# ocrickard/piper-swift

Measured on AMD Instinct MI355X. Metric: audio-sec/wall-sec (RTF^-1) with ms/utterance, Piper VITS en_GB-medium geometry, scale-bench factor, higher is better.
Workload: dtype f32; 1 GPU; medium factor=8: 112 ids, 336 frames, 86016 samples (3.901 s audio) per utterance, 1 utterance per step per GPU; factor=8, phoneme_count=112, frames=336, samples=86016, parallelism=utterance-replicas x1 (one-shot RCCL weight broadcast)

## Files before the change

piper-swift_amd/csrc/conv_lean.hip:

```cpp
#include "conv.h"

namespace ph {
namespace {

typedef float f32x4 __attribute__((ext_vector_type(4)));

struct LeanArgs {
  const float *x, *w, *bias, *res, *skip;
  float *y, *y2;
  const int* len_ptr;
  int len_mul, Lin, Lout, Cout, y_len, nsteps, wn_c;
  int x_row_bytes;
  int x_base_bytes;
  int q_stride;
  int kk_sign;
  int out_ch_base, out_ch_sign;
  int x_batch_bytes;
  long long x_bs, y_bs, y2_bs;
  long long bias_bs;
};

__device__ __forceinline__ float bload(__amdgpu_buffer_rsrc_t r, int voff, int soff) {
  return __builtin_bit_cast(float, __builtin_amdgcn_raw_buffer_load_b32(r, voff, soff, 0));
}

template <int NQ, int MODE>
__global__ __launch_bounds__(512) void conv_k1_kernel(const LeanArgs a, const int nch) {
  __shared__ float red_all[2 * 8 * 4 * 64];
  const int lane = threadIdx.x & 63;
  const int wave = __builtin_amdgcn_readfirstlane((int)(threadIdx.x >> 6));
  const int mt = blockIdx.x, n = blockIdx.z;
  const int lim = a.len_ptr ? min(a.len_ptr[n] * a.len_mul, a.Lout) : a.Lout;
  int ch = blockIdx.y;
// ... 575 lines not shown
    a.out_ch_base = 0; a.out_ch_sign = 1;
    a.x_batch_bytes = (int)(c.x_batch_stride * 4);
    a.x_bs = c.x_batch_stride; a.y_bs = c.y_batch_stride; a.y2_bs = 0; a.bias_bs = 0;
    LnArgs ln{c.ln_gamma, c.ln_beta, c.ln_out, c.ln_eps};
    const dim3 grid((unsigned)ceil_div(c.Cout, 16), (unsigned)ceil_div(c.Lout, 16), (unsigned)c.N);
    if (c.K == 1) hipLaunchKernelGGL((conv_k1_ln_kernel<6>), grid, dim3(512), 0, s, a, ln);
    else if (c.epilogue == EPI_RELU) hipLaunchKernelGGL((conv_k3_ln_kernel<6, EPI_RELU>), grid, dim3(512), 0, s, a, ln);
    else hipLaunchKernelGGL((conv_k3_ln_kernel<6, EPI_STORE>), grid, dim3(512), 0, s, a, ln);
    hipError_t e = hipGetLastError();
    if (e != hipSuccess) PH_FAIL(PIPER_HIP_ERR_LAUNCH, "conv_lean (LayerNorm) launch failed: %s", hipGetErrorString(e));
    return 1;
  }
  if (c.K == 3 && c.w8 && c.Cin == 768 && c.prologue == PRO_NONE && c.epilogue == EPI_STORE && !c.stats_out && !c.gate && c.dil == 1 && c.padL == 1 &&
      c.Lin == c.Lout && c.in_ch_sign == 1 && c.in_ch_base == 0 && c.out_ch_sign == 1 && c.out_ch_base == 0 && c.N <= 65535 && !c.bias_batch_stride) {
    const int mt8 = (int)ceil_div(c.Cout, 8), nch = (int)ceil_div(c.Lout, 16);
    if ((int64_t)mt8 * nch * c.N <= 2 * (int64_t)ctx->num_cus && nch <= 65535 && c.x_batch_stride * 4 < 0x7fffffffLL) {
      LeanArgs a;
      a.x = c.x; a.w = c.w8; a.bias = c.bias; a.res = c.res; a.skip = nullptr; a.y = c.y; a.y2 = nullptr;
      a.len_ptr = c.len_ptr; a.len_mul = c.len_mul;
      a.Lin = c.Lin; a.Lout = c.Lout; a.Cout = c.Cout; a.y_len = c.y_len; a.wn_c = 0; a.nsteps = (c.Cin / 4) * c.K;
      a.x_row_bytes = c.Lin * 4; a.kk_sign = 1; a.x_base_bytes = 0; a.q_stride = 16 * c.Lin; a.out_ch_base = 0; a.out_ch_sign = 1;
      a.x_batch_bytes = (int)(c.x_batch_stride * 4); a.x_bs = c.x_batch_stride; a.y_bs = c.y_batch_stride; a.y2_bs = 0; a.bias_bs = 0;
      const int w_bytes = mt8 * a.nsteps * 128;
      constexpr int NQ = 24;
      const size_t lds = (size_t)(8 * 4 * 64 + 8 * (4 * NQ) * 20) * sizeof(float);
      static bool configured[kMaxDevices] = {};
      if (lds_optin_needed(configured))
        (void)hipFuncSetAttribute((const void*)conv_k3_r8_kernel<NQ>, hipFuncAttributeMaxDynamicSharedMemorySize, 160 * 1024);
      hipLaunchKernelGGL((conv_k3_r8_kernel<NQ>), dim3((unsigned)mt8, (unsigned)nch, (unsigned)c.N), dim3(512), lds, s, a, w_bytes);
      hipError_t e = hipGetLastError();
      if (e != hipSuccess) PH_FAIL(PIPER_HIP_ERR_LAUNCH, "conv_lean (8-row tiles) launch failed: %s", hipGetErrorString(e));
      return 1;
    }
  }
  if (c.K != 1 || c.prologue != PRO_NONE || c.stats_out || !c.w16) return 0;
  if (c.epilogue != EPI_STORE && c.epilogue != EPI_RSUB && c.epilogue != EPI_WN_RES_SKIP && c.epilogue != EPI_WN_SKIP_LAST) return 0;
  if ((c.epilogue == EPI_RSUB || c.epilogue == EPI_WN_RES_SKIP) && !c.res) return 0;
  if (c.Cin % 32 || c.padL != 0 || c.Lin != c.Lout || c.N > 65535 || c.Lout < 1) return 0;
  const int NQ = c.Cin / 32;
  if (NQ != 3 && NQ != 6) return 0;
  if (c.in_ch_sign != 1 && c.in_ch_sign != -1) return 0;
  const int mtiles = (int)ceil_div(c.Cout, 16), nchunks = (int)ceil_div(c.Lout, 16);
  if ((int64_t)mtiles * nchunks * c.N > 64 * (int64_t)ctx->num_cus) return 0;
  if (c.x_batch_stride * 4 >= 0x7fffffffLL) return 0;
  LeanArgs a;
  a.x = c.x; a.w = c.w16; a.bias = c.bias; a.res = c.res; a.skip = c.skip; a.y = c.y; a.y2 = c.y2;
  a.len_ptr = c.len_ptr; a.len_mul = c.len_mul;
  a.Lin = c.Lin; a.Lout = c.Lout; a.Cout = c.Cout; a.y_len = c.y_len; a.wn_c = c.wn_c;
  a.nsteps = c.Cin / 4;
  a.x_row_bytes = c.Lin * 4;
  a.kk_sign = c.in_ch_sign;
  a.x_base_bytes = (c.in_ch_sign > 0 ? c.in_ch_base : c.in_ch_base - 3) * c.Lin * 4;
  a.q_stride = c.in_ch_sign * 16 * c.Lin;
  a.out_ch_base = c.out_ch_base; a.out_ch_sign = c.out_ch_sign;
  a.x_batch_bytes = (int)(c.x_batch_stride * 4);
  a.x_bs = c.x_batch_stride; a.y_bs = c.y_batch_stride; a.y2_bs = c.y2_batch_stride; a.bias_bs = c.bias_batch_stride;
  const dim3 grid((unsigned)mtiles, (unsigned)chunk_groups(ctx, mtiles, nchunks, c.N), (unsigned)c.N);
  const bool ok = NQ == 3 ? launch_lean_nq<3>(s, grid, a, c.epilogue, nchunks) : launch_lean_nq<6>(s, grid, a, c.epilogue, nchunks);
  if (!ok) return 0;
  hipError_t e = hipGetLastError();
  if (e != hipSuccess) PH_FAIL(PIPER_HIP_ERR_LAUNCH, "conv_lean launch failed: %s", hipGetErrorString(e));
  return 1;
}

bool flow_tail_shape_ok(int H, int half) { return H == 192 && half == 96; }

// ... 30 lines not shown
```

piper-swift_amd/csrc/conv_win.h:

```cpp
#pragma once
#include "common.h"

namespace ph {

struct ConvWinArgs {
  const float* x = nullptr;
  const float* x2 = nullptr;
  const float* x3 = nullptr;
  const float* w4 = nullptr;
  const float* bias = nullptr;
  const float* res = nullptr;
  const float* mrf_a = nullptr;
  const float* mrf_b = nullptr;
  float* y = nullptr;
  float pro_alpha = 1.0f;
  float out_alpha = 1.0f;
  int N = 1, Cin = 0, Cout = 0, K = 1, dil = 1, padL = 0;
  int Lin = 0;
  int Lout = 0;
  int y_len = 0;
  int ct_stride = 0, ct_pad = 0;
  const int* len_ptr = nullptr;
  int len_mul = 1;
};

size_t packed_conv_win_floats(int Cout, int Cin, int K);
size_t packed_convt_win_floats(int Cin, int Cout, int K, int stride);
int pack_conv_weights_win(hipStream_t s, const float* w, int Cout, int Cin, int K, float* packed);
int pack_convt_weights_win(hipStream_t s, const float* w, int Cin, int Cout, int K, int stride, int pad, float* packed);

bool conv_win_eligible(int Cout, int Cin, int K, int dil, int padL, int Lin, int Lout);
bool convt_win_eligible(int Cin, int Cout, int K, int stride, int pad, int Lin);

int launch_conv_win(piper_hip_ctx* ctx, hipStream_t s, const ConvWinArgs& a);
constexpr int kWinMulti = 3;
int launch_conv_win_multi(piper_hip_ctx* ctx, hipStream_t s, const ConvWinArgs* convs, int count);

size_t packed_conv_pipe_floats(int Cout, int Cin, int K);
size_t packed_convt_pipe_floats(int Cin, int Cout, int K, int stride);
int pack_conv_weights_pipe(hipStream_t s, const float* w, int Cout, int Cin, int K, float* packed);
int pack_convt_weights_pipe(hipStream_t s, const float* w, int Cin, int Cout, int K, int stride, int pad, float* packed);
bool conv_pipe_eligible(int Cout, int Cin, int K, int dil, int padL, int Lin, int Lout);
bool convt_pipe_eligible(int Cin, int Cout, int K, int stride, int pad, int Lin);
int launch_conv_pipe_multi(piper_hip_ctx* ctx, hipStream_t s, const ConvWinArgs* convs, int count);

struct RbPairArgs {
  const float* x = nullptr;
  float* y = nullptr;
  const float *wa4 = nullptr, *ba = nullptr, *wb4 = nullptr, *bb = nullptr;
  int Ka = 1, dila = 1, Kb = 1, dilb = 1;
  int res_a = 1, res_b_x = 0;
  float alpha = 0.1f;
  int N = 1, C = 0, L = 0;
  const int* len_ptr = nullptr;
  int len_mul = 1;
};
bool rb_pair_eligible(int C, int Ka, int dila, int Kb, int dilb, int L);
int launch_rb_pair_multi(piper_hip_ctx* ctx, hipStream_t s, const RbPairArgs* pairs, int count);

}
```

piper-swift_amd/csrc/voice.hip:

```cpp
#include <algorithm>
#include <cmath>
#include <cstdlib>
#include <chrono>
#include <functional>
#include <memory>

#include "../../include/piper_hip_voice_layout.h"
#include "conv.h"
#include "conv_bf16.h"
#include "conv_win.h"
#include "pcm16.h"
#include "resample.h"
#include "rng.h"
#include "speaker.h"

namespace ph {
int validate_config(const piper_hip_voice_config* c);
int validate_speaker_config(const piper_hip_voice_config* cfg, const piper_hip_speaker_config* sc);
int launch_rel_attention(piper_hip_ctx* ctx, hipStream_t s, const float* q, const float* k, const float* v, const float* ek,
                         const float* ev, float* out, int N, int H, int d, int T, int w, int64_t in_batch_stride,
                         int64_t out_batch_stride, const int* len_ptr);
int rel_attention_split_parts(piper_hip_ctx* ctx, int N, int H, int d, int T, int w);
int launch_rel_attention_split(piper_hip_ctx* ctx, hipStream_t s, const float* q, const float* k, const float* v, const float* ek,
                               const float* ev, float* out, int N, int H, int d, int T, int w, int64_t in_batch_stride,
// ... 99 lines not shown

__global__ void empty_kernel() {}
__global__ void fill_lens_kernel(int* __restrict__ lensT, int* __restrict__ lensF, int T, int F, int n) {
  const int i = blockIdx.x * blockDim.x + threadIdx.x;
  if (i < n) { lensT[i] = T; lensF[i] = F; }
}

__global__ void spin_kernel(unsigned long long ticks) {
  const unsigned long long t0 = __builtin_amdgcn_s_memrealtime();
  while (__builtin_amdgcn_s_memrealtime() - t0 < ticks) __builtin_amdgcn_s_sleep(32);
}

hipError_t stream_wait(hipStream_t q) {
  static const bool park = getenv("PIPER_HIP_NO_SPIN_WAIT") != nullptr;
  if (!park) {
    using clk = std::chrono::steady_clock;
    const auto t0 = clk::now();
    for (;;) {
      const hipError_t e = hipStreamQuery(q);
      if (e != hipErrorNotReady) return e;
      (void)hipGetLastError();
      if (clk::now() - t0 > std::chrono::milliseconds(5)) break;
      for (int i = 0; i < 16; i++) __builtin_ia32_pause();
    }
  }
  return hipStreamSynchronize(q);
}

struct Step {
  std::string name;
  std::function<int(hipStream_t)> run;
  double flops = 0, bytes = 0;
  std::string tag;
  int lane = 0;
  enum Kind { LAUNCH, FORK, JOIN } kind = LAUNCH;
};

struct ConvW {
  const float* w = nullptr;
  const float* w16 = nullptr;
  const float* w16g = nullptr;
  const float* w8 = nullptr;
  const float* w4 = nullptr;
  const float* w5 = nullptr;
  const float* bias = nullptr;
  int Cout = 0, Cin = 0, K = 1;
  bool mfma = false;
};

struct StreamSet {
  hipStream_t stream = nullptr, side[2] = {nullptr, nullptr};
  hipEvent_t ev0 = nullptr, ev1 = nullptr, ev_fork = nullptr, ev_join[2] = {nullptr, nullptr};
};

enum PlanKind : int {
  PLAN_WHOLE = 0,
  PLAN_GENERATOR = 1,
  PLAN_PREDICT = 2,
  PLAN_FROM_STATS = 3,
};

struct RowFormat {
  int rate = 0, enc = PIPER_HIP_ENC_S16;
  float gain = 1.0f;
};

// ... 538 lines not shown
    void* p = nullptr;
    if (rc) return nullptr;
    rc = v->ctx->pool.alloc((n ? n : 1) * sizeof(float), &p);
    if (!rc) { s->owned.push_back(p); s->arena_bytes += (n ? n : 1) * sizeof(float); }
    return (float*)p;
  }
  void* raw(size_t bytes) {
    void* p = nullptr;
    if (rc) return nullptr;
    rc = v->ctx->pool.alloc(bytes ? bytes : 1, &p);
    if (!rc) { s->owned.push_back(p); s->arena_bytes += bytes ? bytes : 1; }
    return p;
  }
};

double conv_bytes(int Cin, int Cout, int K, int64_t L) { return 4.0 * ((double)Cin * L + (double)Cout * L + (double)Cout * Cin * K + Cout); }

double conv_bf16_bytes(const ConvBf16Args& a) {
  const double cols = (double)a.N * a.Lout, out_cols = a.ct_stride > 0 ? cols * a.ct_stride : cols;
  return 2.0 * (a.Cin * cols + (double)a.Cout * a.Cin * a.K) + (a.act ? 2.0 : 0.0) * a.Cout * out_cols +
         ((a.y ? 4.0 : 0.0) + (a.res ? 4.0 : 0.0) + (a.mrf_a ? 8.0 : 0.0)) * a.Cout * out_cols;
}

struct Builder {
  piper_hip_voice* v;
  Slot& s;
  Arena ar;
  const int T, F, NB;
  const int *lensT = nullptr, *lensF = nullptr;
  int lane = 0;
  Builder(piper_hip_voice* v_, Slot& s_, int T_, int F_, int NB_) : v(v_), s(s_), ar{v_, &s_}, T(T_), F(F_), NB(NB_) {}
  Builder(const Builder&) = delete;

  void step(const std::string& name, const char* tag, double flops, double bytes, std::function<int(hipStream_t)> run) {
    Step st;
    st.name = name;
    st.tag = tag;
    st.flops = flops; st.bytes = bytes;
    st.lane = lane;
    st.run = std::move(run);
    s.steps.push_back(std::move(st));
  }
  void mark(const std::string& name, Step::Kind kind) {
    Step st;
    st.name = name;
    st.kind = kind;
    s.steps.push_back(std::move(st));
  }
  void fork(const std::string& name) { mark(name, Step::FORK); }
  void join(const std::string& name) { mark(name, Step::JOIN); }
  void tap(const std::string& name, const float* p, int C, int row, int unit, size_t batch_stride = 0) {
    s.taps[name] = {p, C, row, unit, batch_stride ? batch_stride : (size_t)C * row};
  }

  ConvArgs plain(const float* in, float* out, int Cin_, int Cout_, int L, const int* lens, int mul = 1) const {
    ConvArgs a;
    a.x = in; a.y = out; a.N = NB; a.Lin = L; a.Lout = L; a.x_batch_stride = (int64_t)Cin_ * L; a.y_batch_stride = (int64_t)Cout_ * L;
    a.y_len = L;
    a.len_ptr = lens; a.len_mul = mul;
    return a;
  }

  template <class Args>
  void speaker_bias(Args& a, int row) const {
    if (!v->spk.S || !s.spk_bias) return;
    a.bias = row < 0 ? s.spk_bias : s.spk_bias + row;
    a.bias_batch_stride = row < 0 ? v->cfg.up_initial : v->spk.Ctot;
  }

  void conv(const std::string& name, const ConvW& w, ConvArgs a, int64_t Lout_for_work) {
// ... 13 lines not shown
  void conv_bf16(const std::string& name, const piper_hip_voice::ConvWB& w, ConvBf16Args a, double flops) {
    a.w = w.w; a.Cin = w.Cin; a.Cout = w.Cout; a.K = w.K;
    if (!a.bias) a.bias = w.bias;
    piper_hip_ctx* ctx = v->ctx;
    step(name, "conv_bf16", flops, conv_bf16_bytes(a), [ctx, a](hipStream_t q) { return launch_conv_bf16(ctx, q, a); });
  }

  void conv_bf16_multi(const std::string& name, const piper_hip_voice::ConvWB* const* ws, const ConvBf16Args* args, int count, double flops) {
    struct Pack { ConvBf16Args a[kBf16Multi]; } pk;
    double bytes = 0;
    for (int i = 0; i < count; i++) {
      ConvBf16Args& a = pk.a[i] = args[i];
      const auto& w = *ws[i];
      a.w = w.w; a.bias = w.bias; a.Cin = w.Cin; a.Cout = w.Cout; a.K = w.K;
      bytes += conv_bf16_bytes(a);
    }
    piper_hip_ctx* ctx = v->ctx;
    step(name, "conv_bf16", flops, bytes, [ctx, pk, count](hipStream_t q) { return launch_conv_bf16_multi(ctx, q, pk.a, count); });
  }
};

bool no_merged_rb() { static const bool on = getenv("PIPER_HIP_NO_MERGED_RB") != nullptr; return on; }
bool no_rb_pair() { static const bool on = getenv("PIPER_HIP_NO_RB_PAIR") != nullptr; return on; }

struct GenF32Switches {
  const bool parallel_rb = getenv("PIPER_HIP_PARALLEL_RB") != nullptr;
  const bool use_win = getenv("PIPER_HIP_NO_WIN") == nullptr;
  const bool no_pipe = getenv("PIPER_HIP_NO_PIPE") != nullptr;
  const double pipe_min_flops = [] { const char* e = getenv("PIPER_HIP_PIPE_MIN_GFLOP"); return (e ? atof(e) : 5.0) * 1e9; }();
  const double pipe_ct_min_flops = [] { const char* e = getenv("PIPER_HIP_PIPE_CT_MIN_GFLOP"); return e ? atof(e) * 1e9 : 1e30; }();
  bool pipe_pays(double launch_flops, int Cin, bool ct) const {
    return !no_pipe && launch_flops >= (ct ? pipe_ct_min_flops : pipe_min_flops) && (ct || Cin >= 128);
  }
};
const GenF32Switches& gen_f32_switches() {
  static const GenF32Switches sw;
  return sw;
}


ConvWinArgs win_args(const Builder& b, const ConvW& w, const float* x, const float* res, float* y, int dil, int L, const float* mrf_a = nullptr,
                     const float* mrf_b = nullptr, float out_alpha = 1.0f) {
  ConvWinArgs wa;
  wa.x = x; wa.w4 = w.w4; wa.bias = w.bias; wa.res = res; wa.y = y;
  wa.pro_alpha = 0.1f;
  if (mrf_a) { wa.mrf_a = mrf_a; wa.mrf_b = mrf_b; wa.out_alpha = out_alpha; }
  wa.N = b.NB; wa.Cin = w.Cin; wa.Cout = w.Cout; wa.K = w.K; wa.dil = dil; wa.padL = (w.K * dil - dil) / 2;
  wa.Lin = L; wa.Lout = L; wa.y_len = L;
  wa.len_ptr = b.lensF; wa.len_mul = L / b.F;
  return wa;
}

void add_convt_f32(Builder& b, const std::string& name, const piper_hip_voice::Stage& S, const float* const cur[3], float pro_alpha, float* up,
                   int L) {
  const GenF32Switches& sw = gen_f32_switches();
  piper_hip_ctx* ctx = b.v->ctx;
  const int NB = b.NB, Lo = L * S.stride;
  const double flops = NB * 2.0 * S.Cin * S.Cout * (double)S.K * L;
  const double bytes = NB * 4.0 * ((double)S.Cin * L * (cur[1] ? 3 : 1) + (double)S.Cout * Lo + (double)S.Cin * S.Cout * S.K + S.Cout);
  const bool pipe = sw.use_win && sw.pipe_pays(flops, S.Cin, true) && S.up.w5 && convt_pipe_eligible(S.Cin, S.Cout, S.K, S.stride, S.pad, L);
  if (pipe || (sw.use_win && S.up.w4 && convt_win_eligible(S.Cin, S.Cout, S.K, S.stride, S.pad, L))) {
    ConvWinArgs wa;
    wa.x = cur[0]; wa.x2 = cur[1]; wa.x3 = cur[2]; wa.w4 = pipe ? S.up.w5 : S.up.w4; wa.bias = S.up.bias; wa.y = up;
    wa.pro_alpha = pro_alpha;
    wa.N = NB; wa.Cin = S.Cin; wa.Cout = S.Cout; wa.K = S.K; wa.Lin = L; wa.Lout = L; wa.y_len = Lo;
    wa.ct_stride = S.stride; wa.ct_pad = S.pad;
// ... 281 lines not shown
  }
  const float* cur[3] = {dec0, nullptr, nullptr};
  int L = F;
  for (int u = 0; u < c.n_ups; u++) {
    const auto& S = v->stages[u];
    const int Lo = L * S.stride;
    float* up = ar.f32(B * S.Cout * Lo);
    float* buf[kWinMulti][2];
    float* mid[kWinMulti];
    for (int j = 0; j < c.n_rb; j++) {
      buf[j][0] = ar.f32(B * S.Cout * Lo);
      buf[j][1] = ar.f32(B * S.Cout * Lo);
      mid[j] = c.resblock_type == 1 ? ar.f32(B * S.Cout * Lo) : nullptr;
    }
    if (ar.rc) return ar.rc;
    const std::string p = "dec.s" + std::to_string(u) + ".";
    auto tap_f32 = [&](const std::string& name, const float* ptr) { b.tap(name, ptr, S.Cout, Lo, Lo / F); };
    int held[kWinMulti][2] = {{-1, -1}, {-1, -1}, {-1, -1}};
    auto holds = [&](float* const y[kWinMulti], int di) {
      for (int j = 0; j < kWinMulti; j++) held[j][y[j] == buf[j][1]] = di;
    };
    tap_f32(p + "up", up);
    add_convt_f32(b, p + (cur[1] ? "mrfmean_lrelu_convT" : "lrelu_convT"), S, cur, 0.1f, up, L);
    const float* src[kWinMulti] = {up, up, up};
    auto add_multi = [&](const std::string& name, const ConvW* ws[kWinMulti], const float* const x[kWinMulti],
                         const float* const res[kWinMulti], float* const y[kWinMulti], const int dil[kWinMulti]) {
      struct Pack { ConvWinArgs a[kWinMulti]; } pk;
      double fl = 0, by = 0;
      double launch_fl = 0;
      for (int j = 0; j < kWinMulti; j++) launch_fl += NB * conv_flops(ws[j]->Cout, ws[j]->Cin, ws[j]->K, Lo);
      bool pipe = sw.pipe_pays(launch_fl, ws[0]->Cin, false);
      for (int j = 0; j < kWinMulti; j++)
        pipe = pipe && ws[j]->w5 && conv_pipe_eligible(ws[j]->Cout, ws[j]->Cin, ws[j]->K, dil[j], (ws[j]->K * dil[j] - dil[j]) / 2, Lo, Lo);
      for (int j = 0; j < kWinMulti; j++) {
        const ConvW& w = *ws[j];
        pk.a[j] = win_args(b, w, x[j], res[j], y[j], dil[j], Lo);
        if (pipe) pk.a[j].w4 = w.w5;
        fl += NB * conv_flops(w.Cout, w.Cin, w.K, Lo);
        by += NB * conv_bytes(w.Cin, w.Cout, w.K, Lo);
      }
      if (pipe) b.step(name, "conv_mfma", fl, by, [ctx, pk](hipStream_t q) { return launch_conv_pipe_multi(ctx, q, pk.a, kWinMulti); });
      else b.step(name, "conv_mfma", fl, by, [ctx, pk](hipStream_t q) { return launch_conv_win_multi(ctx, q, pk.a, kWinMulti); });
    };
    const bool no_pair_env = no_rb_pair();
    static const int64_t pair_min_f = [] { const char* e = getenv("PIPER_HIP_RB_PAIR_MIN_F"); return e ? atoll(e) : 128ll; }();
    const bool no_pair = no_pair_env || (int64_t)F * NB < pair_min_f;
    auto add_pair = [&](const std::string& name, int ia, int ib, const int da[kWinMulti], const int db[kWinMulti], bool res_a, bool res_b_x,
                        const float* const x[kWinMulti], float* const y[kWinMulti]) {
      struct Pack { RbPairArgs a[kWinMulti]; } pk;
      double fl = 0, by = 0;
      for (int j = 0; j < kWinMulti; j++) {
        const ConvW &wa = S.rb[j][ia], &wb = S.rb[j][ib];
        if (no_pair || !wa.w4 || !wb.w4 || !wa.bias || !wb.bias || wa.Cin != wa.Cout || wa.Cin != wb.Cin || wb.Cin != wb.Cout ||
            !rb_pair_eligible(wa.Cin, wa.K, da[j], wb.K, db[j], Lo))
          return false;
        RbPairArgs& a = pk.a[j];
        a.x = x[j]; a.y = y[j]; a.wa4 = wa.w4; a.ba = wa.bias; a.wb4 = wb.w4; a.bb = wb.bias;
        a.Ka = wa.K; a.dila = da[j]; a.Kb = wb.K; a.dilb = db[j]; a.res_a = res_a; a.res_b_x = res_b_x; a.alpha = 0.1f;
        a.N = NB; a.C = wa.Cin; a.L = Lo; a.len_ptr = b.lensF; a.len_mul = Lo / F;
        fl += NB * (conv_flops(wa.Cout, wa.Cin, wa.K, Lo) + conv_flops(wb.Cout, wb.Cin, wb.K, Lo));
        by += NB * 4.0 * (2.0 * wa.Cin * (double)Lo + (double)wa.Cin * wa.Cin * (wa.K + wb.K) + 2.0 * wa.Cin);
      }
      b.step(name, "conv_mfma", fl, by, [ctx, pk](hipStream_t q) { return launch_rb_pair_multi(ctx, q, pk.a, kWinMulti); });
      return true;
    };
    for (int di = 0; di < c.rb_n_dil; di++) {
      float* dst[kWinMulti];
      int dil[kWinMulti], one[kWinMulti] = {1, 1, 1};
      const float* none[kWinMulti] = {nullptr, nullptr, nullptr};
      for (int j = 0; j < kWinMulti; j++) { dst[j] = src[j] == buf[j][0] ? buf[j][1] : buf[j][0]; dil[j] = c.rb_dilations[j][di]; }
      const std::string nm = p + "rb012.c" + std::to_string(di);
      if (c.resblock_type == 1 && add_pair(nm + "ab_lrelu_conv_lrelu_conv_res_x3", 2 * di, 2 * di + 1, dil, one, false, true, src, dst)) {
        for (int j = 0; j < kWinMulti; j++) src[j] = dst[j];
        holds(dst, di);
        continue;
// ... 62 lines not shown
    float* m = ar.f32(B * S.Cout * Lo);
    if (ar.rc) return ar.rc;
    const float mean_alpha = (u + 1 == c.n_ups) ? 0.01f : 0.1f;
    auto tap_f32 = [&](const std::string& name, const float* ptr) { b.tap(name, ptr, S.Cout, Lo, Lo / F); };
    tap_f32(p + "up", up);
    tap_f32(p + "mean_lrelu", m);
    for (int j = 0; j < c.n_rb; j++) {
      b.lane = j < 3 ? j : 0;
      const int K = c.rb_kernels[j];
      const float* src = up;
      for (int di = 0; di < c.rb_n_dil; di++) {
        const int dil = c.rb_dilations[j][di];
        const bool lastd = di + 1 == c.rb_n_dil;
        const bool fuse_mean = lastd && j + 1 == c.n_rb && !sw.parallel_rb;
        float* dst = lastd ? (fuse_mean ? m : r[j]) : ((di & 1) ? tmp2[j] : tmp[j]);
        const std::string nm = p + "rb" + std::to_string(j) + ".c" + std::to_string(di);
        if (!fuse_mean && di + 3 >= c.rb_n_dil) tap_f32(nm, dst);
        auto with_mean = [&](ConvArgs a) {
          if (fuse_mean) {
            a.epilogue = EPI_MRF_MEAN;
            a.mrf_a = r[0]; a.mrf_b = r[1]; a.alpha2 = mean_alpha;
          }
          return a;
        };
        auto add_rb = [&](const std::string& name, const ConvW& w, const ConvArgs& a) {
          if (!(sw.use_win && w.w4 && conv_win_eligible(w.Cout, w.Cin, w.K, a.dil, a.padL, Lo, Lo))) {
            b.conv(name, w, a, Lo);
            return;
          }
          ConvWinArgs wa = win_args(b, w, a.x, a.res, a.y, a.dil, Lo, a.epilogue == EPI_MRF_MEAN ? a.mrf_a : nullptr, a.mrf_b, a.alpha2);
          const double flops = NB * conv_flops(w.Cout, w.Cin, w.K, Lo), bytes = NB * conv_bytes(w.Cin, w.Cout, w.K, Lo);
          if (sw.pipe_pays(flops, w.Cin, false) && w.w5 && conv_pipe_eligible(w.Cout, w.Cin, w.K, a.dil, a.padL, Lo, Lo)) {
            wa.w4 = w.w5;
            b.step(name, "conv_mfma", flops, bytes, [ctx, wa](hipStream_t q) { return launch_conv_pipe_multi(ctx, q, &wa, 1); });
          } else {
            b.step(name, "conv_mfma", flops, bytes, [ctx, wa](hipStream_t q) { return launch_conv_win(ctx, q, wa); });
          }
        };
        if (c.resblock_type == 1) {
          add_rb(nm + "a_lrelu_conv", S.rb[j][2 * di], rb_args_f32(b, src, nullptr, mid[j], S.Cout, K, dil, Lo));
          add_rb(nm + (fuse_mean ? "b_lrelu_conv_res_mrfmean" : "b_lrelu_conv_res"), S.rb[j][2 * di + 1],
                 with_mean(rb_args_f32(b, mid[j], src, dst, S.Cout, K, 1, Lo)));
        } else {
          add_rb(nm + (fuse_mean ? "_lrelu_conv_res_mrfmean" : "_lrelu_conv_res"), S.rb[j][di],
                 with_mean(rb_args_f32(b, src, src, dst, S.Cout, K, dil, Lo)));
        }
        src = dst;
      }
    }
    b.lane = 0;
    b.join(p + "join");
    if (sw.parallel_rb)
      add_mrf_mean(b, p + "mrf_mean_lrelu", r[0], r[1], r[2], m, (int64_t)NB * S.Cout * Lo, mean_alpha);
    cur[0] = m; cur[1] = nullptr; cur[2] = nullptr;
    cur_is_mrf = true;
    L = Lo;
  }
  return add_conv_post(b, "dec.conv_post_tanh", cur[0], nullptr, nullptr, PRO_NONE, L);
}

struct FrontBuffers {
  float *x, *x1, *qkv, *att, *att_po, *att_pml, *y, *ff, *stats, *zp, *zflip, *zp_tap, *h, *acts, *skip;
  int att_parts;
};

int build_encoder(Builder& b, const FrontBuffers& fb, bool for_predictor) {
  piper_hip_voice* v = b.v;
  Arena& ar = b.ar;
  const int T = b.T, NB = b.NB;
// ... 2927 lines not shown
  if (n_samples) *n_samples = (int64_t)v->attached[0]->h_F[0] * v->hop;
  return PIPER_HIP_OK;
}

PH_EXPORT int piper_hip_voice_tap(piper_hip_voice* v, int slot, const char* name, float* host, size_t max_floats,
                                  size_t* n_floats) {
  if (!v || !name) PH_FAIL(PIPER_HIP_ERR_ARG, "null argument");
  Slot* sp = slot_plan(v, slot);
  if (!sp) PH_FAIL(PIPER_HIP_ERR_ARG, "slot %d is not prepared", slot);
  const Slot& owner = *sp;
  std::string full(name);
  Slot* tp = sp;
  if (full.compare(0, 8, "predict:") == 0) {
    full.erase(0, 8);
    tp = nullptr;
    for (auto& p : v->plans)
      if (p->built && p->kind == PLAN_PREDICT && p->T == owner.T && p->NB == owner.NB && p->prec == v->precision) { tp = p.get(); break; }
    if (!tp) PH_FAIL(PIPER_HIP_ERR_ARG, "tap '%s': no predictor plan of %d ids x %d items is cached", name, owner.T, owner.NB);
  }
  Slot& s = *tp;
  const size_t at = full.find('@');
  const std::string tensor_name = full.substr(0, at), step_name = at == std::string::npos ? std::string() : full.substr(at + 1);
  if (at != std::string::npos && tensor_name.empty() && step_name == "steps") {
    std::string all;
    for (const Step& st : s.steps)
      if (st.kind == Step::LAUNCH) all += st.name + "\n";
    if (n_floats) *n_floats = all.size();
    if (host) {
      if (max_floats < all.size()) PH_FAIL(PIPER_HIP_ERR_SHAPE, "tap buffer too small");
      for (size_t i = 0; i < all.size(); i++) host[i] = (float)(unsigned char)all[i];
    }
    return PIPER_HIP_OK;
  }
  auto it = s.taps.find(tensor_name);
  if (it == s.taps.end()) PH_FAIL(PIPER_HIP_ERR_ARG, "unknown tap '%s'", name);
  const Slot::Tap& t = it->second;
  int upto = -1;
  if (at != std::string::npos) {
    if (s.kind == PLAN_GENERATOR) PH_FAIL(PIPER_HIP_ERR_UNSUPPORTED, "tap '%s': a generator-only window plan keeps no inputs to replay from", name);
    if (owner.bounded_pending) PH_FAIL(PIPER_HIP_ERR_UNSUPPORTED, "tap '%s': the slot's frame counts are still on the device (collect first)", name);
    for (int i = 0; i < (int)s.steps.size() && upto < 0; i++)
      if (s.steps[i].kind == Step::LAUNCH && s.steps[i].name == step_name) upto = i;
    if (upto < 0) PH_FAIL(PIPER_HIP_ERR_ARG, "tap '%s': the schedule has no step '%s'", name, step_name.c_str());
  }
  auto item_len = [&](int b) { return (size_t)(t.unit < 0 ? t.row : t.unit == 0 ? owner.h_T[b] : owner.h_F[b] * t.unit); };
  size_t total = 0;
  for (int b = 0; b < s.NB; b++) total += (size_t)t.C * item_len(b);
  if (n_floats) *n_floats = total;
  if (host) {
    if (max_floats < total) PH_FAIL(PIPER_HIP_ERR_SHAPE, "tap buffer too small");
    PH_HIP(hipSetDevice(v->ctx->device), PIPER_HIP_ERR_UNAVAILABLE);
    if (tp != sp) {
      PH_HIP(stream_wait(owner.set.stream), PIPER_HIP_ERR_LAUNCH);
      const int rc = slot_init(v, s);
      if (rc) return rc;
    }
    const hipStream_t q = s.set.stream;
    PH_HIP(stream_wait(q), PIPER_HIP_ERR_LAUNCH);
    auto run_range = [&](int from, int to) -> int {
      for (int i = from; i < to; i++)
        if (s.steps[i].kind == Step::LAUNCH) {
          const int rc = s.steps[i].run(q);
          if (rc) return rc;
        }
      PH_HIP(hipGetLastError(), PIPER_HIP_ERR_LAUNCH);
      PH_HIP(stream_wait(q), PIPER_HIP_ERR_LAUNCH);
// ... 161 lines not shown
```

piper-swift_amd/python/piper_hip/__init__.py:

```python
import ctypes as C
import os

import numpy as np

_HERE = os.path.dirname(os.path.abspath(__file__))
LIB_PATH = os.path.normpath(os.path.join(_HERE, "..", "..", "lib", "libpiper_hip.so"))
LIB_NORT_PATH = os.path.normpath(os.path.join(_HERE, "..", "..", "lib", "libpiper_hip_nort.so"))



class ExecutionError(RuntimeError):
    code = None


class ShapeMismatch(ExecutionError):
    code = -1


class TypeMismatch(ExecutionError):
    code = -2


class UnsupportedOp(ExecutionError):
    code = -3
# ... 1528 lines not shown
        rate = src if rate is None else int(rate)
        u, _k = self._utt(phonemeIDs, durations, noise, noiseScale)
        n = int(self.lib.piper_hip_voice_num_samples(self.voice, C.byref(u)))
        if rate != src:
            n = resample_count(src, rate, n)
        out = np.empty(max(n, 1), np.uint8)
        got = C.c_int64()
        prm = PcmParams(float(gain), int(bool(normalize)))
        _check(self.lib.piper_hip_voice_synthesize_g711(self.voice, C.byref(u), C.byref(prm), _law(law), rate, out.ctypes.data_as(c_u8p), n,
                                                        C.byref(got)))
        self._keep.pop(0, None)
        return out[:got.value]

    def peaks(self, slot):
        nb = self.lib.piper_hip_voice_batch_size(self.voice, slot)
        out = np.empty(max(nb, 1), np.float32)
        _check(self.lib.piper_hip_voice_peaks(self.voice, slot, out.ctypes.data_as(c_f32p), nb))
        return out[:nb]

    def tap(self, slot, name, max_floats=None):
        n = C.c_size_t()
        if max_floats is None:
            _check(self.lib.piper_hip_voice_tap(self.voice, slot, name.encode(), None, 0, C.byref(n)))
            max_floats = max(int(n.value), 1)
        out = np.empty(max_floats, np.float32)
        _check(self.lib.piper_hip_voice_tap(self.voice, slot, name.encode(), out.ctypes.data_as(c_f32p), max_floats,
                                            C.byref(n)))
        return out[:n.value]

    def steps(self, slot, predict=False):
        raw = self.tap(slot, ("predict:" if predict else "") + "@steps")
        return bytes(raw.astype(np.uint8)).decode().split("\n")[:-1]

    def last_gpu_ms(self, slot):
        ms = C.c_double()
        _check(self.lib.piper_hip_voice_last_gpu_ms(self.voice, slot, C.byref(ms)))
        return ms.value

    def time_subset(self, slot, name_filter, iters=20):
        us, n, fl, by = C.c_double(), C.c_int(), C.c_double(), C.c_double()
        _check(self.lib.piper_hip_voice_time_subset(self.voice, slot, name_filter.encode(), iters, C.byref(us), C.byref(n),
                                                    C.byref(fl), C.byref(by)))
        return us.value, n.value, fl.value, by.value

    def profile(self, slot, iters=5, max_entries=512):
        arr = (KernelStat * max_entries)()
        n = C.c_int()
        _check(self.lib.piper_hip_voice_profile(self.voice, slot, iters, arr, max_entries, C.byref(n)))
        return [dict(name=a.name.decode(), avg_us=a.avg_us, flops=a.flops, bytes=a.bytes) for a in arr[:n.value]]
```

Measured before the change: 5802 audio-sec/wall-sec.

## Add lean MFMA kernel for small-L 128-channel resblock dilated convs

Adds a new conv_rb_lean kernel for 128-channel K=3/5/7 dilated resblock convolutions at small sequence lengths. It keeps weights in registers, splits the input-channel reduction across 8 waves with an LDS reduction, prefetches the next column chunk while computing, and fuses leaky-ReLU and the residual add. Grid slots are spread across the three convs in proportion to K so that CUs stay filled. The kernel is routed into the generator resblock multi-conv and single-conv paths, and into conv_lean when a call fits. A kernel-name tap is also added for introspection. The aim is to cut launch/latency-bound overhead of the window kernel on short sequences, at the cost of more kernel variants and an extra cross-wave reduction.

Result: no change. 5857 audio-sec/wall-sec (median of 6 runs) (+1.0%).

```diff
diff --git a/piper-swift_amd/csrc/conv_lean.hip b/piper-swift_amd/csrc/conv_lean.hip
--- a/piper-swift_amd/csrc/conv_lean.hip
+++ b/piper-swift_amd/csrc/conv_lean.hip
@@ -1,4 +1,5 @@
 #include "conv.h"
+#include "conv_win.h"
 
 namespace ph {
 namespace {
@@ -640,6 +641,19 @@
       if (e != hipSuccess) PH_FAIL(PIPER_HIP_ERR_LAUNCH, "conv_lean (8-row tiles) launch failed: %s", hipGetErrorString(e));
       return 1;
     }
+  }
+  if (c.K >= 3 && c.w16 && c.Cin == c.Cout && (c.prologue == PRO_NONE || (c.prologue == PRO_LRELU && c.alpha > 0.0f && c.alpha <= 1.0f)) &&
+      c.epilogue == EPI_STORE && !c.stats_out && c.dil >= 1 && c.Lin == c.Lout && c.y_len == c.Lout && c.padL == (c.K - 1) * c.dil / 2 &&
+      c.in_ch_sign == 1 && c.in_ch_base == 0 && c.out_ch_sign == 1 && c.out_ch_base == 0 && !c.bias_batch_stride &&
+      c.x_batch_stride == (int64_t)c.Cin * c.Lin && c.y_batch_stride == (int64_t)c.Cout * c.Lout &&
+      rb_lean_eligible(ctx, c.Cin, c.K, c.dil, c.Lout, c.N, 1)) {
+    ConvWinArgs wa;
+    wa.x = c.x; wa.w4 = c.w16; wa.bias = c.bias; wa.res = c.res; wa.y = c.y;
+    wa.pro_alpha = c.prologue == PRO_LRELU ? c.alpha : 1.0f;
+    wa.N = c.N; wa.Cin = c.Cin; wa.Cout = c.Cout; wa.K = c.K; wa.dil = c.dil; wa.padL = c.padL;
+    wa.Lin = c.Lin; wa.Lout = c.Lout; wa.y_len = c.y_len; wa.len_ptr = c.len_ptr; wa.len_mul = c.len_mul;
+    const int rc = launch_rb_lean_multi(ctx, s, &wa, 1);
+    return rc ? rc : 1;
   }
   if (c.K != 1 || c.prologue != PRO_NONE || c.stats_out || !c.w16) return 0;
   if (c.epilogue != EPI_STORE && c.epilogue != EPI_RSUB && c.epilogue != EPI_WN_RES_SKIP && c.epilogue != EPI_WN_SKIP_LAST) return 0;
diff --git a/piper-swift_amd/csrc/conv_rb_lean.hip b/piper-swift_amd/csrc/conv_rb_lean.hip
--- /dev/null
+++ b/piper-swift_amd/csrc/conv_rb_lean.hip
@@ -0,0 +1,218 @@
+#include "conv.h"
+#include "conv_win.h"
+
+namespace ph {
+namespace {
+
+typedef float f32x4 __attribute__((ext_vector_type(4)));
+
+constexpr int kC = 128;
+constexpr int kRowTiles = kC / 16;
+constexpr int kMaxReach = 72;
+constexpr int kExchFloats = 2 * 8 * 4 * 64;
+
+struct RbLeanConv {
+  const float *x, *w, *bias, *res;
+  float* y;
+  int K, dil;
+};
+
+struct RbLeanArgs {
+  RbLeanConv c[kWinMulti];
+  const int* len_ptr;
+  int len_mul, L, pitch, adjacent, x_batch_bytes;
+  int gend[kWinMulti];
+  float alpha;
+  long long bs;
+};
+
+__device__ __forceinline__ float bload(__amdgpu_buffer_rsrc_t r, int voff, int soff) {
+  return __builtin_bit_cast(float, __builtin_amdgcn_raw_buffer_load_b32(r, voff, soff, 0));
+}
+
+template <int K, int NP, bool RES_LATE>
+__device__ __forceinline__ void rb_lean_body(const RbLeanArgs& a, const RbLeanConv& cv, const int mt, const int y, const int ngroups, const int nch,
+                                             float* sm) {
+  constexpr int NQ = 4, NS = NQ * K;
+  constexpr int OOB = 0x7fffffff, PAST = 0x3fffffff;
+  const int lane = threadIdx.x & 63;
+  const int wave = __builtin_amdgcn_readfirstlane((int)(threadIdx.x >> 6));
+  const int n = blockIdx.z, L = a.L, pitch = a.pitch;
+  const int Lv = a.len_ptr ? min(a.len_ptr[n] * a.len_mul, L) : L;
+  int ch, ch_end, ch_step;
+  if (a.adjacent) {
+    const int per = (nch + ngroups - 1) / ngroups;
+    ch = y * per; ch_end = min(ch + per, nch); ch_step = 1;
+  } else {
+    ch = y; ch_end = nch; ch_step = ngroups;
+  }
+  if (ch >= ch_end || ch * 16 >= Lv) return;
+  const int j = lane & 15, kk = lane >> 4;
+  const __amdgpu_buffer_rsrc_t rx = __builtin_amdgcn_make_buffer_rsrc((void*)(cv.x + (long long)n * a.bs), 0, a.x_batch_bytes, 0x00020000);
+  const float* wa = cv.w + (((long long)mt * (kC / 4 * K) + wave * NS) << 6) + lane;
+  float av[NS];
+#pragma unroll
+  for (int s = 0; s < NS; s++) av[s] = wa[s * 64];
+  const int dil = cv.dil, reach = (K - 1) * dil, pad = reach >> 1, W = 16 + reach;
+  const int sbase = wave * 16 * L * 4;
+  float xa[NP][NQ];
+  auto request = [&](int t0) {
+#pragma unroll
+    for (int p = 0; p < NP; p++) {
+      const int c = 16 * p + j, pos = t0 - pad + c;
+      const int voff = (c < W && pos >= 0 && pos < Lv) ? (kk * L + pos) * 4 : OOB;
+#pragma unroll
+      for (int i = 0; i < NQ; i++) xa[p][i] = bload(rx, voff, sbase + i * 16 * L);
+    }
+  };
+  request(ch * 16);
+  float* xs = sm + kExchFloats + wave * (16 * pitch);
+  float* xc = xs + kk * pitch + j;
+  const int row = 16 * mt + 4 * kk + wave;
+  const float bias = (wave < 4 && cv.bias) ? cv.bias[row] : 0.0f;
+  const long long orow = (long long)n * a.bs + (long long)row * L;
+  const bool has_res = cv.res != nullptr;
+  const __amdgpu_buffer_rsrc_t rr = __builtin_amdgcn_make_buffer_rsrc((void*)((has_res ? cv.res : cv.x) + (long long)n * a.bs), 0, a.x_batch_bytes, 0x00020000);
+  const float alpha = a.alpha;
+  for (int it = 0;; it++) {
+    const int t0 = ch * 16;
+    const int nxt = ch + ch_step;
+    const bool more = nxt < ch_end && nxt * 16 < Lv;
+#pragma unroll
+    for (int p = 0; p < NP; p++) {
+#pragma unroll
+      for (int i = 0; i < NQ; i++) xc[4 * i * pitch + 16 * p] = fmaxf(xa[p][i], alpha * xa[p][i]);
+    }
+    __builtin_amdgcn_fence(__ATOMIC_RELEASE, "wavefront");
+    __builtin_amdgcn_wave_barrier();
+    __builtin_amdgcn_fence(__ATOMIC_ACQUIRE, "wavefront");
+    const int col = t0 + j;
+    const bool fin = wave < 4 && col < Lv;
+    float rv = 0.0f;
+    if constexpr (!RES_LATE) rv = bload(rr, (fin && has_res) ? (row * L + col) * 4 : OOB, 0);
+    request(more ? nxt * 16 : PAST);
+    __builtin_amdgcn_sched_barrier(0);
+    f32x4 acc = {0.0f, 0.0f, 0.0f, 0.0f};
+#pragma unroll
+    for (int qi = 0; qi < NQ; qi++)
+#pragma unroll
+      for (int k = 0; k < K; k++) acc = __builtin_amdgcn_mfma_f32_16x16x4f32(av[qi * K + k], xc[4 * qi * pitch + k * dil], acc, 0, 0, 0);
+    float* red = sm + (it & 1) * (8 * 4 * 64);
+#pragma unroll
+    for (int r = 0; r < 4; r++) red[(wave * 4 + r) * 64 + lane] = acc[r];
+    __syncthreads();
+    if (wave < 4) {
+      float v = bias;
+      float part[8];
+#pragma unroll
+      for (int s = 0; s < 8; s++) part[s] = red[(s * 4 + wave) * 64 + lane];
+      if constexpr (RES_LATE) rv = bload(rr, (fin && has_res) ? (row * L + col) * 4 : OOB, 0);
+#pragma unroll
+      for (int s = 0; s < 8; s++) v += part[s];
+      if (fin) cv.y[orow + col] = has_res ? v + rv : v;
+    }
+    if (!more) break;
+    ch = nxt;
+  }
+}
+
+template <int NPMAX, bool RES_LATE>
+__global__ __launch_bounds__(512) void conv_rb_lean_kernel(const RbLeanArgs a, const int nch) {
+  extern __shared__ __attribute__((aligned(16))) float sm[];
+  const int mt = blockIdx.x, gy = blockIdx.y;
+  RbLeanConv cv = a.c[0];
+  int y0 = 0, y1 = a.gend[0];
+  if (gy >= a.gend[0]) { cv = a.c[1]; y0 = a.gend[0]; y1 = a.gend[1]; }
+  if (gy >= a.gend[1]) { cv = a.c[2]; y0 = a.gend[1]; y1 = a.gend[2]; }
+  const int np = (16 + (cv.K - 1) * cv.dil + 15) >> 4;
+  const int cls = np <= 2 ? 2 : np <= 3 ? 3 : 6;
+#define PH_RB_LEAN_CASE(KK, PP) \
+  case KK * 8 + PP: rb_lean_body<KK, PP, RES_LATE>(a, cv, mt, gy - y0, y1 - y0, nch, sm); break
+  switch (cv.K * 8 + cls) {
+    PH_RB_LEAN_CASE(3, 2); PH_RB_LEAN_CASE(5, 2); PH_RB_LEAN_CASE(7, 2);
+    PH_RB_LEAN_CASE(3, 3); PH_RB_LEAN_CASE(5, 3); PH_RB_LEAN_CASE(7, 3);
+    default:
+      if constexpr (NPMAX > 3) {
+        switch (cv.K) {
+          case 3: rb_lean_body<3, 6, RES_LATE>(a, cv, mt, gy - y0, y1 - y0, nch, sm); break;
+          case 5: rb_lean_body<5, 6, RES_LATE>(a, cv, mt, gy - y0, y1 - y0, nch, sm); break;
+          default: rb_lean_body<7, 6, RES_LATE>(a, cv, mt, gy - y0, y1 - y0, nch, sm); break;
+        }
+      }
+  }
+#undef PH_RB_LEAN_CASE
+}
+
+bool rb_lean_off() {
+  static const bool off = getenv("PIPER_HIP_NO_RB_LEAN") != nullptr;
+  return off;
+}
+
+int piece_class(int K, int dil) {
+  const int np = (16 + (K - 1) * dil + 15) / 16;
+  return np <= 2 ? 2 : np <= 3 ? 3 : 6;
+}
+
+}
+
+bool rb_lean_eligible(piper_hip_ctx* ctx, int C, int K, int dil, int L, int N, int count) {
+  if (rb_lean_off()) return false;
+  if (C != kC || (K != 3 && K != 5 && K != 7) || dil < 1 || (K - 1) * dil > kMaxReach || L < 1 || N < 1 || N > 65535) return false;
+  if (count < 1 || count > kWinMulti) return false;
+  const int64_t nch = ceil_div(L, 16);
+  return (int64_t)count * kRowTiles * nch * N <= 64 * (int64_t)ctx->num_cus && (int64_t)C * L * 4 < 0x7fffffffLL;
+}
+
+int launch_rb_lean_multi(piper_hip_ctx* ctx, hipStream_t s, const ConvWinArgs* convs, int count) {
+  if (count < 1 || count > kWinMulti) PH_FAIL(PIPER_HIP_ERR_ARG, "rb_lean: %d convs in one launch", count);
+  const ConvWinArgs& c0 = convs[0];
+  RbLeanArgs a{};
+  int np = 1;
+  for (int i = 0; i < count; i++) {
+    const ConvWinArgs& c = convs[i];
+    if (!rb_lean_eligible(ctx, c.Cin, c.K, c.dil, c.Lout, c.N, count) || c.Cout != kC || c.Lin != c.Lout || c.y_len != c.Lout ||
+        c.padL != (c.K - 1) * c.dil / 2 || c.N != c0.N || c.Lout != c0.Lout || c.len_ptr != c0.len_ptr || c.len_mul != c0.len_mul ||
+        c.pro_alpha != c0.pro_alpha || !(c.pro_alpha > 0.0f && c.pro_alpha <= 1.0f) || c.x2 || c.x3 || c.mrf_a || c.mrf_b || c.out_alpha != 1.0f ||
+        c.ct_stride || !c.x || !c.w4 || !c.y)
+      PH_FAIL(PIPER_HIP_ERR_UNSUPPORTED, "rb_lean: conv %d (C=%d→%d K=%d dil=%d L=%d N=%d) not covered", i, c.Cin, c.Cout, c.K, c.dil, c.Lout, c.N);
+    a.c[i] = RbLeanConv{c.x, c.w4, c.bias, c.res, c.y, c.K, c.dil};
+    np = std::max(np, piece_class(c.K, c.dil));
+  }
+  for (int i = count; i < kWinMulti; i++) a.c[i] = a.c[0];
+  a.len_ptr = c0.len_ptr; a.len_mul = c0.len_mul; a.L = c0.Lout; a.alpha = c0.pro_alpha;
+  a.pitch = 16 * (np | 1);
+  a.x_batch_bytes = kC * c0.Lout * 4; a.bs = (long long)kC * c0.Lout;
+  static const bool adjacent = getenv("PIPER_HIP_RB_LEAN_ADJACENT") != nullptr;
+  static const bool res_late = getenv("PIPER_HIP_RB_LEAN_RES_EARLY") == nullptr;
+  static const bool even = getenv("PIPER_HIP_RB_LEAN_EVEN") != nullptr;
+  a.adjacent = adjacent;
+  const size_t lds = (size_t)(kExchFloats + 8 * 16 * a.pitch) * sizeof(float);
+  const int per_cu = (int)std::min<size_t>(2, (160 * 1024) / lds);
+  const int nch = (int)ceil_div(c0.Lout, 16);
+  const int64_t slots = std::max<int64_t>(count, (int64_t)per_cu * ctx->num_cus / ((int64_t)kRowTiles * c0.N));
+  int ksum = 0, gtot = 0;
+  for (int i = 0; i < count; i++) ksum += even ? 1 : convs[i].K;
+  for (int i = 0; i < kWinMulti; i++) {
+    if (i < count) gtot += (int)std::max<int64_t>(1, std::min<int64_t>(nch, slots * (even ? 1 : convs[i].K) / ksum));
+    a.gend[i] = gtot;
+  }
+  const dim3 grid((unsigned)kRowTiles, (unsigned)gtot, (unsigned)c0.N);
+  if (np <= 3) {
+    if (res_late) hipLaunchKernelGGL((conv_rb_lean_kernel<3, true>), grid, dim3(512), lds, s, a, nch);
+    else hipLaunchKernelGGL((conv_rb_lean_kernel<3, false>), grid, dim3(512), lds, s, a, nch);
+  } else {
+    static bool configured[kMaxDevices] = {};
+    if (lds_optin_needed(configured)) {
+      (void)hipFuncSetAttribute((const void*)conv_rb_lean_kernel<6, true>, hipFuncAttributeMaxDynamicSharedMemorySize, 160 * 1024);
+      (void)hipFuncSetAttribute((const void*)conv_rb_lean_kernel<6, false>, hipFuncAttributeMaxDynamicSharedMemorySize, 160 * 1024);
+    }
+    if (res_late) hipLaunchKernelGGL((conv_rb_lean_kernel<6, true>), grid, dim3(512), lds, s, a, nch);
+    else hipLaunchKernelGGL((conv_rb_lean_kernel<6, false>), grid, dim3(512), lds, s, a, nch);
+  }
+  hipError_t e = hipGetLastError();
+  if (e != hipSuccess) PH_FAIL(PIPER_HIP_ERR_LAUNCH, "conv_rb_lean launch failed: %s", hipGetErrorString(e));
+  return PIPER_HIP_OK;
+}
+
+}
+namespace ph { namespace { PH_WARM(conv_rb_lean, (conv_rb_lean_kernel<3, false>)); } }
diff --git a/piper-swift_amd/csrc/conv_win.h b/piper-swift_amd/csrc/conv_win.h
--- a/piper-swift_amd/csrc/conv_win.h
+++ b/piper-swift_amd/csrc/conv_win.h
@@ -44,6 +44,9 @@
 bool convt_pipe_eligible(int Cin, int Cout, int K, int stride, int pad, int Lin);
 int launch_conv_pipe_multi(piper_hip_ctx* ctx, hipStream_t s, const ConvWinArgs* convs, int count);
 
+bool rb_lean_eligible(piper_hip_ctx* ctx, int C, int K, int dil, int L, int N, int count);
+int launch_rb_lean_multi(piper_hip_ctx* ctx, hipStream_t s, const ConvWinArgs* convs, int count);
+
 struct RbPairArgs {
   const float* x = nullptr;
   float* y = nullptr;
diff --git a/piper-swift_amd/csrc/voice.hip b/piper-swift_amd/csrc/voice.hip
--- a/piper-swift_amd/csrc/voice.hip
+++ b/piper-swift_amd/csrc/voice.hip
@@ -155,6 +155,7 @@
   std::function<int(hipStream_t)> run;
   double flops = 0, bytes = 0;
   std::string tag;
+  std::string kernel;
   int lane = 0;
   enum Kind { LAUNCH, FORK, JOIN } kind = LAUNCH;
 };
@@ -759,10 +760,11 @@
   Builder(piper_hip_voice* v_, Slot& s_, int T_, int F_, int NB_) : v(v_), s(s_), ar{v_, &s_}, T(T_), F(F_), NB(NB_) {}
   Builder(const Builder&) = delete;
 
-  void step(const std::string& name, const char* tag, double flops, double bytes, std::function<int(hipStream_t)> run) {
+  void step(const std::string& name, const char* tag, double flops, double bytes, std::function<int(hipStream_t)> run, const char* kernel = nullptr) {
     Step st;
     st.name = name;
     st.tag = tag;
+    st.kernel = kernel ? kernel : tag;
     st.flops = flops; st.bytes = bytes;
     st.lane = lane;
     st.run = std::move(run);
@@ -842,6 +844,8 @@
   bool pipe_pays(double launch_flops, int Cin, bool ct) const {
     return !no_pipe && launch_flops >= (ct ? pipe_ct_min_flops : pipe_min_flops) && (ct || Cin >= 128);
   }
+  const int64_t rb_lean_min_cols = [] { const char* e = getenv("PIPER_HIP_RB_LEAN_MIN_COLS"); return e ? atoll(e) : 0ll; }();
+  bool rb_lean_pays(int64_t cols) const { return cols >= rb_lean_min_cols; }
 };
 const GenF32Switches& gen_f32_switches() {
   static const GenF32Switches sw;
@@ -1189,15 +1193,20 @@
       bool pipe = sw.pipe_pays(launch_fl, ws[0]->Cin, false);
       for (int j = 0; j < kWinMulti; j++)
         pipe = pipe && ws[j]->w5 && conv_pipe_eligible(ws[j]->Cout, ws[j]->Cin, ws[j]->K, dil[j], (ws[j]->K * dil[j] - dil[j]) / 2, Lo, Lo);
+      bool lean = !pipe && sw.rb_lean_pays((int64_t)Lo * NB);
+      for (int j = 0; j < kWinMulti; j++)
+        lean = lean && ws[j]->w16 && ws[j]->Cout == ws[j]->Cin && rb_lean_eligible(ctx, ws[j]->Cin, ws[j]->K, dil[j], Lo, NB, kWinMulti);
       for (int j = 0; j < kWinMulti; j++) {
         const ConvW& w = *ws[j];
         pk.a[j] = win_args(b, w, x[j], res[j], y[j], dil[j], Lo);
         if (pipe) pk.a[j].w4 = w.w5;
+        if (lean) pk.a[j].w4 = w.w16;
         fl += NB * conv_flops(w.Cout, w.Cin, w.K, Lo);
         by += NB * conv_bytes(w.Cin, w.Cout, w.K, Lo);
       }
-      if (pipe) b.step(name, "conv_mfma", fl, by, [ctx, pk](hipStream_t q) { return launch_conv_pipe_multi(ctx, q, pk.a, kWinMulti); });
-      else b.step(name, "conv_mfma", fl, by, [ctx, pk](hipStream_t q) { return launch_conv_win_multi(ctx, q, pk.a, kWinMulti); });
+      if (pipe) b.step(name, "conv_mfma", fl, by, [ctx, pk](hipStream_t q) { return launch_conv_pipe_multi(ctx, q, pk.a, kWinMulti); }, "conv_pipe_kernel");
+      else if (lean) b.step(name, "conv_mfma", fl, by, [ctx, pk](hipStream_t q) { return launch_rb_lean_multi(ctx, q, pk.a, kWinMulti); }, "conv_rb_lean_kernel");
+      else b.step(name, "conv_mfma", fl, by, [ctx, pk](hipStream_t q) { return launch_conv_win_multi(ctx, q, pk.a, kWinMulti); }, "conv_win_kernel");
     };
     const bool no_pair_env = no_rb_pair();
     static const int64_t pair_min_f = [] { const char* e = getenv("PIPER_HIP_RB_PAIR_MIN_F"); return e ? atoll(e) : 128ll; }();
@@ -1326,9 +1335,12 @@
           const double flops = NB * conv_flops(w.Cout, w.Cin, w.K, Lo), bytes = NB * conv_bytes(w.Cin, w.Cout, w.K, Lo);
           if (sw.pipe_pays(flops, w.Cin, false) && w.w5 && conv_pipe_eligible(w.Cout, w.Cin, w.K, a.dil, a.padL, Lo, Lo)) {
             wa.w4 = w.w5;
-            b.step(name, "conv_mfma", flops, bytes, [ctx, wa](hipStream_t q) { return launch_conv_pipe_multi(ctx, q, &wa, 1); });
+            b.step(name, "conv_mfma", flops, bytes, [ctx, wa](hipStream_t q) { return launch_conv_pipe_multi(ctx, q, &wa, 1); }, "conv_pipe_kernel");
+          } else if (a.epilogue != EPI_MRF_MEAN && w.w16 && w.Cout == w.Cin && sw.rb_lean_pays((int64_t)Lo * NB) && rb_lean_eligible(ctx, w.Cin, w.K, a.dil, Lo, NB, 1)) {
+            wa.w4 = w.w16;
+            b.step(name, "conv_mfma", flops, bytes, [ctx, wa](hipStream_t q) { return launch_rb_lean_multi(ctx, q, &wa, 1); }, "conv_rb_lean_kernel");
           } else {
-            b.step(name, "conv_mfma", flops, bytes, [ctx, wa](hipStream_t q) { return launch_conv_win(ctx, q, wa); });
+            b.step(name, "conv_mfma", flops, bytes, [ctx, wa](hipStream_t q) { return launch_conv_win(ctx, q, wa); }, "conv_win_kernel");
           }
         };
         if (c.resblock_type == 1) {
@@ -4322,6 +4334,17 @@
     }
     return PIPER_HIP_OK;
   }
+  if (at != std::string::npos && tensor_name.empty() && step_name == "kernels") {
+    std::string all;
+    for (const Step& st : s.steps)
+      if (st.kind == Step::LAUNCH) all += st.name + "\t" + st.kernel + "\n";
+    if (n_floats) *n_floats = all.size();
+    if (host) {
+      if (max_floats < all.size()) PH_FAIL(PIPER_HIP_ERR_SHAPE, "tap buffer too small");
+      for (size_t i = 0; i < all.size(); i++) host[i] = (float)(unsigned char)all[i];
+    }
+    return PIPER_HIP_OK;
+  }
   auto it = s.taps.find(tensor_name);
   if (it == s.taps.end()) PH_FAIL(PIPER_HIP_ERR_ARG, "unknown tap '%s'", name);
   const Slot::Tap& t = it->second;
diff --git a/piper-swift_amd/python/piper_hip/__init__.py b/piper-swift_amd/python/piper_hip/__init__.py
--- a/piper-swift_amd/python/piper_hip/__init__.py
+++ b/piper-swift_amd/python/piper_hip/__init__.py
@@ -1584,6 +1584,10 @@
         raw = self.tap(slot, ("predict:" if predict else "") + "@steps")
         return bytes(raw.astype(np.uint8)).decode().split("\n")[:-1]
 
+    def step_kernels(self, slot, predict=False):
+        raw = self.tap(slot, ("predict:" if predict else "") + "@kernels")
+        return [tuple(ln.split("\t")) for ln in bytes(raw.astype(np.uint8)).decode().split("\n")[:-1]]
+
     def last_gpu_ms(self, slot):
         ms = C.c_double()
         _check(self.lib.piper_hip_voice_last_gpu_ms(self.voice, slot, C.byref(ms)))
```
